# aras-p/UnityGaussianSplatting

Measured on AMD Instinct MI355X. Metric: Msplats/s rendered (sort+view+composite+resolve), bicycle-sized synthetic 6,131,954 splats, 1200x797, Medium; ms/frame in ms_per_step, higher is better.
Workload: dtype f32; 1 GPU; bicycle-sized synthetic 6,131,954 splats, 1200x797, Medium; sort_mode=visible_in_flight, frames_in_flight=2, frames_in_flight_impl=library, splats=6131954, views=1, views_per_rank=1, blend=exact, sort_nth_frame=1, tile_pairs_P=4376060, tile=32x16, visible_splats=1563698, parallelism=single GPU, rccl_ranks=0

## Files before the change

### unitygaussiansplatting_amd/csrc/gs_device_math.h

```cpp
#pragma once
#include <stdint.h>

#if defined(__HIPCC__)
#include <hip/hip_runtime.h>
#include <hip/hip_fp16.h>
#define GS_HD __host__ __device__ __forceinline__
#else
#include <cmath>
#include <cstring>
#define GS_HD inline
#endif

#ifndef GS_CULL_EXTENT
#define GS_CULL_EXTENT 2.8285f
#endif

namespace gsm {

struct AssetView {
    const uint8_t* pos;
    const uint8_t* other;
    const uint8_t* color;
    const uint8_t* sh;
    const uint8_t* chunk;
// ... 505 lines not shown
                    BoxRec& rec, int& x0, int& x1, int& y0, int& y1) {
    const float det = Inverse3(B, rec.inv);
    bool ok = finite32(det) && det != 0.0f;
    for (int k = 0; k < 9; ++k) ok = ok && finite32(rec.inv[k]);
    if (!ok || !(al > 0.0f)) return false;
    const float dx = rc.ox - c[0], dy = rc.oy - c[1], dz = rc.oz - c[2];
    for (int k = 0; k < 3; ++k) rec.lo[k] = fmaf(rec.inv[k * 3 + 2], dz, fmaf(rec.inv[k * 3 + 1], dy, rec.inv[k * 3] * dx));
    rec.r = r; rec.g = g; rec.b = bl; rec.a = det < 0.0f ? -al : al;
    float minx = 3.0e38f, maxx = -3.0e38f, miny = 3.0e38f, maxy = -3.0e38f;
    bool behind = false;
    for (int corner = 0; corner < 8; ++corner) {
        const float lx = (corner & 1) ? 1.0f : -1.0f, ly = (corner & 2) ? 1.0f : -1.0f, lz = (corner & 4) ? 1.0f : -1.0f;
        const float wx = c[0] + fmaf(B[2], lz, fmaf(B[1], ly, B[0] * lx)), wy = c[1] + fmaf(B[5], lz, fmaf(B[4], ly, B[3] * lx)),
                    wz = c[2] + fmaf(B[8], lz, fmaf(B[7], ly, B[6] * lx));
        const float cx = mrow(vp, 0, wx, wy, wz), cy = mrow(vp, 1, wx, wy, wz), cw = mrow(vp, 3, wx, wy, wz);
        if (!(cw > 1.0e-6f)) { behind = true; continue; }
        const float sx = fmaf(0.5f * (cx / cw), rc.W, 0.5f * rc.W), sy = fmaf(-0.5f * (cy / cw), rc.H, 0.5f * rc.H);
        minx = fminf(minx, sx); maxx = fmaxf(maxx, sx); miny = fminf(miny, sy); maxy = fmaxf(maxy, sy);
    }
    if (behind || !(finite32(minx) && finite32(maxx) && finite32(miny) && finite32(maxy))) { x0 = 0; y0 = 0; x1 = (int)rc.W - 1; y1 = (int)rc.H - 1; return true; }
    const float fx0 = fmaxf(floorf(minx) - 1.0f, 0.0f), fx1 = fminf(ceilf(maxx) + 1.0f, rc.W - 1.0f);
    const float fy0 = fmaxf(floorf(miny) - 1.0f, 0.0f), fy1 = fminf(ceilf(maxy) + 1.0f, rc.H - 1.0f);
    if (!(fx0 <= fx1 && fy0 <= fy1)) return false;
    x0 = (int)fx0; x1 = (int)fx1; y0 = (int)fy0; y1 = (int)fy1;
    return true;
}

GS_HD bool IsSplatCut(const EditView& e, float px, float py, float pz) {
    bool finalCut = false;
    for (uint32_t i = 0; i < e.cutoutCount; ++i) {
        const uint32_t* c = e.cutouts + i * 17u;
        const uint32_t tf = c[16];
        const uint32_t type = tf & 0xFFu;
        if (type == 0xFFu) continue;
        const bool invert = (tf & 0xFF00u) != 0;
        float m[12];
#pragma unroll
        for (int k = 0; k < 12; ++k) m[k] = u2f(c[k]);
        const float cx = mrow(m, 0, px, py, pz), cy = mrow(m, 1, px, py, pz), cz = mrow(m, 2, px, py, pz);
        if (type == 0u) { if (dot3f(cx, cy, cz, cx, cy, cz) <= 1.0f) return invert; }
        if (type == 1u) { if (fabsf(cx) <= 1.0f && fabsf(cy) <= 1.0f && fabsf(cz) <= 1.0f) return invert; }
        finalCut = finalCut || !invert;
    }
    return finalCut;
}

struct ViewPartial {
    ViewData view;
    V4 col;
    V3 shMin, shMax;
    float wx, wy, wz;
    uint64_t otherEnd;
    bool shLerp;
    bool front;
    bool culled;
};

GS_HD void CalcViewGeom(const AssetView& a, const FrameConsts& P, const EditView& E, uint32_t idx, ViewPartial& vp, bool allowCull = false,
                        bool outputsOnlyIfDrawn = false) {
    ViewData& view = vp.view;
    if (!outputsOnlyIfDrawn) {
        view.pos[0] = view.pos[1] = view.pos[2] = view.pos[3] = 0.0f;
        view.axis1[0] = view.axis1[1] = view.axis2[0] = view.axis2[1] = 0.0f;
        view.color[0] = view.color[1] = 0u;
        vp.shLerp = false; vp.otherEnd = 0u;
        vp.shMin = { 0, 0, 0 }; vp.shMax = { 0, 0, 0 }; vp.col = { 0, 0, 0, 0 };
    }
    vp.front = false; vp.culled = false;

    V3 pos = LoadVec(a.pos, (uint64_t)idx * vecStride(a.posFmt), a.posFmt);
    const uint32_t ci = idx >> 8;
    const bool chunked = ci < a.chunkCount;
    ChunkRaw ck;
    if (chunked) {
        ck = LoadChunk(a.chunk, ci);
        pos.x = lerpf(u2f(ck.w[4]), u2f(ck.w[5]), pos.x);
        pos.y = lerpf(u2f(ck.w[6]), u2f(ck.w[7]), pos.y);
        pos.z = lerpf(u2f(ck.w[8]), u2f(ck.w[9]), pos.z);
    }
    const float wx = mrow(P.o2w, 0, pos.x, pos.y, pos.z), wy = mrow(P.o2w, 1, pos.x, pos.y, pos.z), wz = mrow(P.o2w, 2, pos.x, pos.y, pos.z);
    vp.wx = wx; vp.wy = wy; vp.wz = wz;
    view.pos[0] = mrow(P.vp, 0, wx, wy, wz);
    view.pos[1] = mrow(P.vp, 1, wx, wy, wz);
    view.pos[2] = mrow(P.vp, 2, wx, wy, wz);
    view.pos[3] = mrow(P.vp, 3, wx, wy, wz);
    if (E.deletedBits && ((E.deletedBits[idx >> 5] >> (idx & 31u)) & 1u)) view.pos[3] = 0.0f;
    if (E.cutoutCount && IsSplatCut(E, pos.x, pos.y, pos.z)) view.pos[3] = 0.0f;
    if (view.pos[3] <= 0.0f) return;
    vp.front = true;

    uint32_t otherStride = 4 + vecStride(a.scaleFmt);
    if (a.shFmt > 3) otherStride += 2;
    const uint64_t otherAddr = (uint64_t)idx * otherStride;
    vp.otherEnd = otherAddr + otherStride;
    V3 scale = LoadVec(a.other, otherAddr + 4, a.scaleFmt);
    if (chunked) {
        scale.x = lerpf(f16tof32(ck.w[10]), f16tof32(ck.w[10] >> 16), scale.x);
        scale.y = lerpf(f16tof32(ck.w[11]), f16tof32(ck.w[11] >> 16), scale.y);
        scale.z = lerpf(f16tof32(ck.w[12]), f16tof32(ck.w[12] >> 16), scale.z);
        scale.x *= scale.x; scale.y *= scale.y; scale.z *= scale.z;
        scale.x *= scale.x; scale.y *= scale.y; scale.z *= scale.z;
        scale.x *= scale.x; scale.y *= scale.y; scale.z *= scale.z;
    }
    const float ss2 = P.splatScale * P.splatScale;

    float vx = mrow(P.mv, 0, pos.x, pos.y, pos.z), vy = mrow(P.mv, 1, pos.x, pos.y, pos.z);
    const float vz = mrow(P.mv, 2, pos.x, pos.y, pos.z);
    const float limX = P.limX, limY = P.limY, focal = P.focal;
    const float rz = 1.0f / vz;
    vx = fminf(fmaxf(vx * rz, -limX), limX) * vz;
    vy = fminf(fmaxf(vy * rz, -limY), limY) * vz;
    const float rzz = rz * rz;
    const float J00 = focal * rz, J02 = -(focal * vx) * rzz;
    const float J11 = J00, J12 = -(focal * vy) * rzz;
    const float T00 = fmaf(J02, P.mv[8], J00 * P.mv[0]), T01 = fmaf(J02, P.mv[9], J00 * P.mv[1]), T02 = fmaf(J02, P.mv[10], J00 * P.mv[2]);
    const float T10 = fmaf(J12, P.mv[8], J11 * P.mv[4]), T11 = fmaf(J12, P.mv[9], J11 * P.mv[5]), T12 = fmaf(J12, P.mv[10], J11 * P.mv[6]);

    if (allowCull) {
        const float w = view.pos[3];
        if (!(w >= P.nearClip && w <= P.farClip)) { vp.culled = true; return; }
        const float smax = fmaxf(fmaxf(fabsf(scale.x), fabsf(scale.y)), fabsf(scale.z));
        const float t2 = dot3f(T00, T01, T02, T00, T01, T02) + dot3f(T10, T11, T12, T10, T11, T12);
        const float lam = fmaf(t2 * (1.1f * ss2), smax * smax, 0.6f);
#if defined(__HIP_DEVICE_COMPILE__)
        const float rad = fmaf(GS_CULL_EXTENT * 1.05f, __builtin_amdgcn_sqrtf(2.0f * lam), 2.0f);
#else
        const float rad = fmaf(GS_CULL_EXTENT * 1.05f, sqrtf(2.0f * lam), 2.0f);
#endif
        const float invw = 1.0f / w;
        const float cx = fmaf(0.5f * (view.pos[0] * invw), P.screenW, 0.5f * P.screenW);
        const float cy = fmaf(-0.5f * (view.pos[1] * invw), P.screenH, 0.5f * P.screenH);
        if (cx - rad > P.screenW || cx + rad < 0.0f || cy - rad > P.screenH || cy + rad < 0.0f) { vp.culled = true; return; }
    }

    const V4 q = DecodeRotation(LoadUInt(a.other, otherAddr));

    V4 col = LoadColorTexel(a, idx);

    if (chunked) {
        col.x = lerpf(f16tof32(ck.w[0]), f16tof32(ck.w[0] >> 16), col.x);
        col.y = lerpf(f16tof32(ck.w[1]), f16tof32(ck.w[1] >> 16), col.y);
        col.z = lerpf(f16tof32(ck.w[2]), f16tof32(ck.w[2] >> 16), col.z);
        col.w = lerpf(f16tof32(ck.w[3]), f16tof32(ck.w[3] >> 16), col.w);
        col.w = InvSquareCentered01(col.w);
        vp.shMin = { f16tof32(ck.w[13]), f16tof32(ck.w[14]), f16tof32(ck.w[15]) };
        vp.shMax = { f16tof32(ck.w[13] >> 16), f16tof32(ck.w[14] >> 16), f16tof32(ck.w[15] >> 16) };
        vp.shLerp = a.shFmt > 0 && a.shFmt <= 3;
    } else {
        vp.shLerp = false; vp.shMin = { 0, 0, 0 }; vp.shMax = { 0, 0, 0 };
    }
    vp.col = col;

    const float x = q.x, y = q.y, z = q.z, w = q.w;
    const float r00 = fmaf(-2.0f, y * y + z * z, 1.0f), r01 = 2.0f * fmaf(x, y, -(w * z)), r02 = 2.0f * fmaf(x, z, w * y);
    const float r10 = 2.0f * fmaf(x, y, w * z), r11 = fmaf(-2.0f, fmaf(x, x, z * z), 1.0f), r12 = 2.0f * fmaf(y, z, -(w * x));
    const float r20 = 2.0f * fmaf(x, z, -(w * y)), r21 = 2.0f * fmaf(y, z, w * x), r22 = fmaf(-2.0f, fmaf(x, x, y * y), 1.0f);
    const float m00 = r00 * scale.x, m01 = r01 * scale.y, m02 = r02 * scale.z;
    const float m10 = r10 * scale.x, m11 = r11 * scale.y, m12 = r12 * scale.z;
    const float m20 = r20 * scale.x, m21 = r21 * scale.y, m22 = r22 * scale.z;
    const float c00 = dot3f(m00, m01, m02, m00, m01, m02) * ss2, c01 = dot3f(m00, m01, m02, m10, m11, m12) * ss2, c02 = dot3f(m00, m01, m02, m20, m21, m22) * ss2;
    const float c11 = dot3f(m10, m11, m12, m10, m11, m12) * ss2, c12 = dot3f(m10, m11, m12, m20, m21, m22) * ss2, c22 = dot3f(m20, m21, m22, m20, m21, m22) * ss2;

    const float VT00 = dot3f(c00, c01, c02, T00, T01, T02), VT01 = dot3f(c00, c01, c02, T10, T11, T12);
    const float VT10 = dot3f(c01, c11, c12, T00, T01, T02), VT11 = dot3f(c01, c11, c12, T10, T11, T12);
    const float VT20 = dot3f(c02, c12, c22, T00, T01, T02), VT21 = dot3f(c02, c12, c22, T10, T11, T12);
    const float cov00 = dot3f(T00, T01, T02, VT00, VT10, VT20) + 0.3f;
    const float cov01 = dot3f(T00, T01, T02, VT01, VT11, VT21);
    const float cov11 = dot3f(T10, T11, T12, VT01, VT11, VT21) + 0.3f;

    const float mid = 0.5f * (cov00 + cov11);
    const float hx = (cov00 - cov11) / 2.0f;
    const float radius = sqrtf(dot2f(hx, cov01, hx, cov01));
    const float lambda1 = mid + radius;
    const float lambda2 = fmaxf(mid - radius, 0.1f);
    float dvx = cov01, dvy = lambda1 - cov00;
    const float invLen = 1.0f / sqrtf(dot2f(dvx, dvy, dvx, dvy));
    dvx *= invLen; dvy *= invLen;
    dvy = -dvy;
    const float s1 = fminf(sqrtf(2.0f * lambda1), 4096.0f), s2 = fminf(sqrtf(2.0f * lambda2), 4096.0f);
    view.axis1[0] = s1 * dvx; view.axis1[1] = s1 * dvy;
    view.axis2[0] = s2 * dvy; view.axis2[1] = s2 * (-dvx);

    const float al = fminf(col.w * P.opacityScale, 65000.0f);
    view.color[1] = f32tof16(al);
}

template <class SHSource>
GS_HD void CalcViewColor(const AssetView& a, const FrameConsts& P, uint32_t idx, ViewPartial& vp, SHSource& shsrc) {
    ViewData& view = vp.view;
    const V4 col = vp.col;
    const V3 shMin = vp.shMin, shMax = vp.shMax;
    const bool shLerp = vp.shLerp;
    const float wx = vp.wx, wy = vp.wy, wz = vp.wz;
    const float dwx = P.camx - wx, dwy = P.camy - wy, dwz = P.camz - wz;
    float ox = mrow3(P.w2o, 0, dwx, dwy, dwz), oy = mrow3(P.w2o, 1, dwx, dwy, dwz), oz = mrow3(P.w2o, 2, dwx, dwy, dwz);
    const float invN = 1.0f / sqrtf(dot3f(ox, oy, oz, ox, oy, oz));
    ox *= invN; oy *= invN; oz *= invN;
    const float dx = -ox, dy = -oy, dz = -oz;

    const bool onlySH = P.shOnly != 0;
    F2 rg = onlySH ? F2{ 0.5f, 0.5f } : F2{ col.x, col.y };
    float b = onlySH ? 0.5f : col.z;
    if (P.shOrder >= 1) {
        uint32_t shIndex = idx;
        if (a.shFmt > 3) shIndex = LoadUShort(a.other, vp.otherEnd - 2);
        shsrc.begin(a.sh + (uint64_t)shIndex * shStrideOf(a.shFmt), a.shFmt);
        const F2 minRG = { shMin.x, shMin.y }, dRG = F2{ shMax.x, shMax.y } - minRG;
        const float minB = shMin.z, dB = shMax.z - shMin.z;
        auto SHK = [&](int k) -> RGB {
            RGB s = shsrc.load_rgb(k);
            if (shLerp) { s.rg = fma2(s.rg, dRG, minRG); s.b = fmaf(s.b, dB, minB); }
            return s;
        };
        auto MUL = [](float w, const RGB& s) -> RGB { return { F2{ w, w } * s.rg, w * s.b }; };
        auto FMA = [](float w, const RGB& s, const RGB& acc) -> RGB { return { fma2(F2{ w, w }, s.rg, acc.rg), fmaf(w, s.b, acc.b) }; };
        {
            const RGB s1v = SHK(1), s2v = SHK(2), s3v = SHK(3);
            RGB t = MUL(dy, RGB{ -s1v.rg, -s1v.b });
            t = FMA(dz, s2v, t);
            t = FMA(dx, RGB{ -s3v.rg, -s3v.b }, t);
            rg = fma2(F2{ GS_SH_C1, GS_SH_C1 }, t.rg, rg); b = fmaf(GS_SH_C1, t.b, b);
        }
        if (P.shOrder >= 2) {
            const float xx = dx * dx, yy = dy * dy, zz = dz * dz;
            const float xy = dx * dy, yz = dy * dz, xz = dx * dz;
            {
                const float b4 = 1.0925484f * xy, b5 = -1.0925484f * yz, b6 = 0.3153916f * (fmaf(2.0f, zz, -xx) - yy),
                            b7 = -1.0925484f * xz, b8 = 0.5462742f * (xx - yy);
                RGB acc = MUL(b4, SHK(4));
                acc = FMA(b5, SHK(5), acc);
                acc = FMA(b6, SHK(6), acc);
                acc = FMA(b7, SHK(7), acc);
                acc = FMA(b8, SHK(8), acc);
                rg += acc.rg; b += acc.b;
            }
            if (P.shOrder >= 3) {
                const float b9 = (-0.5900436f * dy) * fmaf(3.0f, xx, -yy);
                const float b10 = (2.8906114f * xy) * dz;
                const float b11 = (-0.4570458f * dy) * (fmaf(4.0f, zz, -xx) - yy);
                const float b12 = (0.3731763f * dz) * (fmaf(2.0f, zz, -3.0f * xx) - 3.0f * yy);
                const float b13 = (-0.4570458f * dx) * (fmaf(4.0f, zz, -xx) - yy);
                const float b14 = (1.4453057f * dz) * (xx - yy);
                const float b15 = (-0.5900436f * dx) * fmaf(-3.0f, yy, xx);
                RGB acc = MUL(b9, SHK(9));
                acc = FMA(b10, SHK(10), acc);
// ... 37 lines not shown
constexpr uint32_t kAlphaWindowLo = kAlphaThresholdBits - kAlphaWindow / 2u;
GS_HD float Exp2Det(float y) {
    const float n = rintf(y);
    const float f = y - n;
    float p = 1.525273380405984e-05f;
    p = fmaf(p, f, 1.5403530393381608e-04f);
    p = fmaf(p, f, 1.3333558146428443e-03f);
    p = fmaf(p, f, 9.618129107628477e-03f);
    p = fmaf(p, f, 5.550410866482158e-02f);
    p = fmaf(p, f, 2.402265069591007e-01f);
    p = fmaf(p, f, 6.931471805599453e-01f);
    p = fmaf(p, f, 1.0f);
    return ldexpf(p, (int)n);
}
GS_HD float DecideAlpha(float alphaNative, float y, float a, bool& live) {
    const uint32_t u = f2u(alphaNative) - kAlphaWindowLo;
    if (u < kAlphaWindow) {
        const float ad = fminf(fmaxf(Exp2Det(y) * a, 0.0f), 1.0f);
        live = ad >= u2f(kAlphaThresholdBits);
        return ad;
    }
    live = (int32_t)u >= (int32_t)kAlphaWindow;
    return alphaNative;
}

GS_HD float LogDet(float x) {
    const uint32_t u = f2u(x);
    float e = (float)((int)(u >> 23) - 127);
    float m = u2f((u & 0x7fffffu) | 0x3f800000u);
    if (m > 1.41421356f) { m *= 0.5f; e += 1.0f; }
    const float t = (m - 1.0f) / (m + 1.0f);
    const float t2 = t * t;
    const float p = fmaf(t2, fmaf(t2, fmaf(t2, 1.0f / 7.0f, 0.2f), 1.0f / 3.0f), 1.0f);
    return fmaf(e, 0.69314718f, (2.0f * t) * p);
}

GS_HD bool BlockMayTouch(float bcx, float bcy, float half, float cx, float cy, float u1x, float u1y, float u2x, float u2y, float r2) {
    const float dx = bcx - cx, dy = bcy - cy;
    const float d1 = fabsf(fmaf(dy, u1y, dx * u1x)) - half * (fabsf(u1x) + fabsf(u1y));
    const float d2 = fabsf(fmaf(dy, u2y, dx * u2x)) - half * (fabsf(u2x) + fabsf(u2y));
    const float m1 = fmaxf(d1, 0.0f), m2 = fmaxf(d2, 0.0f);
    return (m1 <= 2.001f) && (m2 <= 2.001f) && (fmaf(m2, m2, m1 * m1) <= r2);
}

struct SplatFootprint {
    float cx, cy;
    int x0, x1, y0, y1;
};
GS_HD void PackPixelRect(const SplatFootprint& fp, uint32_t& rx, uint32_t& ry) {
    rx = (uint32_t)fp.x0 | ((uint32_t)fp.y0 << 16);
    ry = (uint32_t)(fp.x1 + 1) | ((uint32_t)(fp.y1 + 1) << 16);
}

GS_HD bool PrepareSplat(const ViewData& v, float W, float H, float nearClip, float farClip, SplatFootprint& fp) {
    fp.x0 = 1; fp.x1 = 0; fp.y0 = 1; fp.y1 = 0; fp.cx = 0.0f; fp.cy = 0.0f;
    const float w = v.pos[3];
    const float a = f16tof32(v.color[1]);
    const int drawable = (int)(w > 0.0f) & (int)(w >= nearClip) & (int)(w <= farClip) & (int)finite32(v.axis1[0]) & (int)finite32(v.axis1[1]) &
                         (int)finite32(v.axis2[0]) & (int)finite32(v.axis2[1]) & (int)(a >= 1.0f / 255.0f);
    if (!drawable) return false;
    const float invw = 1.0f / w;
    const float cx = fmaf(0.5f * (v.pos[0] * invw), W, 0.5f * W);
    const float cy = fmaf(-0.5f * (v.pos[1] * invw), H, 0.5f * H);
    const float a1x = v.axis1[0], a1y = v.axis1[1], a2x = v.axis2[0], a2y = v.axis2[1];
    const float d1 = dot2f(a1x, a1y, a1x, a1y), d2 = dot2f(a2x, a2y, a2x, a2y);
    const int inv1ok = (int)((f2u(d1) - 0x00200001u) <= (0x7f800000u - 0x00200001u)), inv2ok = (int)((f2u(d2) - 0x00200001u) <= (0x7f800000u - 0x00200001u));
    fp.cx = cx; fp.cy = cy;
    if (!((int)finite32(cx) & (int)finite32(cy) & inv1ok & inv2ok)) return false;
    const float exr = 2.0f * (fabsf(a1x) + fabsf(a2x)), eyr = 2.0f * (fabsf(a1y) + fabsf(a2y));
    const float slack = 0.01f;
    int x0, x1, y0, y1;
    PixRange(fp.cx, exr + slack, W, x0, x1);
    PixRange(fp.cy, eyr + slack, H, y0, y1);
    if (x0 > x1 || y0 > y1) return false;
    const float r2 = fmaf(LogDet(255.0f * a), 1.0001f, 1.0e-3f);
    const float rr = sqrtf(fmaxf(r2, 0.0f));
    const float exe = rr * sqrtf(dot2f(a1x, a2x, a1x, a2x)), eye = rr * sqrtf(dot2f(a1y, a2y, a1y, a2y));
    PixRange(fp.cx, fminf(exr, exe) + slack, W, x0, x1);
    PixRange(fp.cy, fminf(eyr, eye) + slack, H, y0, y1);
    if (x0 > x1 || y0 > y1) return true;
    fp.x0 = x0; fp.x1 = x1; fp.y0 = y0; fp.y1 = y1;
    return true;
}

}
```

### unitygaussiansplatting_amd/csrc/gs_raster.hip

```cpp
#include "gs_common.h"
#include <cstdlib>

namespace gs {

namespace {

struct RasterConsts {
    float W, H, nearClip, farClip;
    uint32_t tilesX, tilesY, width, height;
};

constexpr unsigned long long BFLAG_AGG = 1ull << 62, BFLAG_INCL = 2ull << 62, BVAL_MASK = (1ull << 62) - 1ull;
constexpr uint32_t BIN_SPIN_LIMIT = 1u << 24;

__device__ __forceinline__ float rl(float x, int b) { return __int_as_float(__builtin_amdgcn_readlane(__float_as_int(x), b)); }

__device__ __forceinline__ uint32_t wave_incl_scan_u32(uint32_t v) {
#define GS_DPP(x, ctrl, rowmask) (uint32_t)__builtin_amdgcn_update_dpp(0, (int)(x), ctrl, rowmask, 0xf, false)
    v += GS_DPP(v, 0x111, 0xf);
    v += GS_DPP(v, 0x112, 0xf);
    v += GS_DPP(v, 0x114, 0xf);
    v += GS_DPP(v, 0x118, 0xf);
    v += GS_DPP(v, 0x142, 0xa);
    v += GS_DPP(v, 0x143, 0xc);
// ... 599 lines not shown
        for (uint32_t t = tid; t < kBinTileCounters; t += kEmitThreads) {
            const uint32_t c = s_tile[t];
            if (c) {
                atomicAdd(&s_hist[t & digitMask], c);
                if (PASSES >= 2) atomicAdd(&s_hist[256 + ((t >> digitBits) & digitMask)], c);
            }
        }
        __syncthreads();
    }
    uint32_t* myHist = pairHist + (bid % histCopies) * (uint32_t)kHistStride;
    for (int j = tid; j < PASSES * 256; j += kEmitThreads) {
        const uint32_t c = s_hist[j];
        if (c) atomicAdd(&myHist[j], c);
    }
}

__global__ __launch_bounds__(256) void tile_ranges_kernel(const uint32_t* __restrict__ pairKeys, const uint32_t* nPtr,
                                                          uint32_t* __restrict__ tileStart, uint32_t* __restrict__ tileEnd, uint32_t numTiles) {
    GS_CHAIN_PRIORITY();
    const uint32_t n = *nPtr;
    const uint32_t octs = (n + 7u) >> 3;
    for (uint32_t q = blockIdx.x * 256u + threadIdx.x; q < octs; q += gridDim.x * 256u) {
        const uint32_t j0 = q << 3;
        const uint4 ka = ((const uint4*)pairKeys)[2u * q], kb = ((const uint4*)pairKeys)[2u * q + 1u];
        const uint32_t k[10] = { j0 ? pairKeys[j0 - 1u] : 0xffffffffu, ka.x, ka.y, ka.z, ka.w, kb.x, kb.y, kb.z, kb.w,
                                 (j0 + 8u < n) ? pairKeys[j0 + 8u] : 0xffffffffu };
#pragma unroll
        for (int c = 0; c < 8; ++c) {
            const uint32_t j = j0 + (uint32_t)c;
            if (j >= n) break;
            const uint32_t t = k[c + 1];
            if (t >= numTiles) continue;
            if (j == 0 || k[c] != t) tileStart[t] = j;
            if (j == n - 1 || k[c + 2] != t) tileEnd[t] = j + 1;
        }
    }
}

__device__ __forceinline__ float mix_mul_lo(uint32_t h, float x) {
    float d;
    asm("v_fma_mix_f32 %0, %1, %2, 0 op_sel_hi:[1,0,0]" : "=v"(d) : "v"(h), "v"(x));
    return d;
}
__device__ __forceinline__ float mix_mul_hi(uint32_t h, float x) {
    float d;
    asm("v_fma_mix_f32 %0, %1, %2, 0 op_sel:[1,0,0] op_sel_hi:[1,0,0]" : "=v"(d) : "v"(h), "v"(x));
    return d;
}
__device__ __forceinline__ float mix_mul_lo_sat_after_trans(uint32_t h, float x) {
    float d;
    asm("s_nop 0\n\tv_fma_mix_f32 %0, %1, %2, 0 op_sel_hi:[1,0,0] clamp" : "=v"(d) : "v"(h), "v"(x));
    return d;
}
__device__ __forceinline__ float mix_one_minus_hi(uint32_t h) {
    float d;
    asm("v_fma_mix_f32 %0, %1, -1.0, 1.0 op_sel:[1,0,0] op_sel_hi:[1,0,0]" : "=v"(d) : "v"(h));
    return d;
}
__device__ __forceinline__ void mix_blend4(uint32_t& rg, uint32_t& ba, float pr, float pg, float pb, float pa, float t) {
    asm("v_fma_mixlo_f16 %0, %2, %6, %0 op_sel_hi:[0,0,1]\n\t"
        "v_fma_mixlo_f16 %1, %4, %6, %1 op_sel_hi:[0,0,1]\n\t"
        "v_fma_mixhi_f16 %0, %3, %6, %0 op_sel:[0,0,1] op_sel_hi:[0,0,1]\n\t"
        "v_fma_mixhi_f16 %1, %5, %6, %1 op_sel:[0,0,1] op_sel_hi:[0,0,1]"
        : "+v"(rg), "+v"(ba) : "v"(pr), "v"(pg), "v"(pb), "v"(pa), "v"(t));
}

__device__ __forceinline__ float half_lo(uint32_t u) { return (float)__builtin_bit_cast(_Float16, (unsigned short)(u & 0xffffu)); }
__device__ __forceinline__ float half_hi(uint32_t u) { return (float)__builtin_bit_cast(_Float16, (unsigned short)(u >> 16)); }
template <int MODE> struct PixelAcc;
template <> struct PixelAcc<0> {
    uint32_t rg, ba;
    __device__ __forceinline__ void load(uint2 d) { rg = d.x; ba = d.y; }
    __device__ __forceinline__ void blend(uint32_t c0, uint32_t c1, float alpha) {
        const float t = mix_one_minus_hi(ba);
        mix_blend4(rg, ba, mix_mul_hi(c0, alpha), mix_mul_lo(c0, alpha), mix_mul_hi(c1, alpha), alpha, t);
    }
    __device__ __forceinline__ void blend_src(float pr, float pg, float pb, float pa) { const float t = mix_one_minus_hi(ba); mix_blend4(rg, ba, pr, pg, pb, pa, t); }
    __device__ __forceinline__ bool finished() const { return (ba >> 16) == 0x3c00u; }
    __device__ __forceinline__ bool saturated() const { return false; }
    __device__ __forceinline__ uint2 pack() const { return make_uint2(rg, ba); }
};
template <> struct PixelAcc<1> {
    float r, g, b, a;
    __device__ __forceinline__ void load(uint2 d) {
        r = gsm::f16tof32(d.x); g = gsm::f16tof32(d.x >> 16); b = gsm::f16tof32(d.y); a = gsm::f16tof32(d.y >> 16);
    }
    __device__ __forceinline__ void blend(uint32_t c0, uint32_t c1, float alpha) {
        const float t = 1.0f - a;
        r = fmaf(mix_mul_hi(c0, alpha), t, r); g = fmaf(mix_mul_lo(c0, alpha), t, g); b = fmaf(mix_mul_hi(c1, alpha), t, b);
        a = fmaf(alpha, t, a);
    }
    __device__ __forceinline__ void blend_src(float pr, float pg, float pb, float pa) { const float t = 1.0f - a; r = fmaf(pr, t, r); g = fmaf(pg, t, g); b = fmaf(pb, t, b); a = fmaf(pa, t, a); }
    __device__ __forceinline__ bool finished() const { return (1.0f - a) < (1.0f / 4096.0f); }
    __device__ __forceinline__ bool saturated() const { return (1.0f - a) < (1.0f / 4096.0f); }
    __device__ __forceinline__ uint2 pack() const {
        uint2 o;
        o.x = gsm::f32tof16(r) | (gsm::f32tof16(g) << 16);
        o.y = gsm::f32tof16(b) | (gsm::f32tof16(a) << 16);
        return o;
    }
};

typedef uint32_t u4v __attribute__((ext_vector_type(4)));

#ifdef GS_BLEND_STATS
__device__ unsigned long long g_blendStats[8];
#define GS_STAT(i, v) do { if (lane == 0) atomicAdd(&g_blendStats[i], (unsigned long long)(v)); } while (0)
#else
#define GS_STAT(i, v) do { } while (0)
#endif
#ifdef GS_BLEND_TL
__device__ unsigned long long g_blendTl[8192 * 8];
#endif
template <int MODE, bool DEPTH, int TWL, int THL>
__global__ __launch_bounds__(64 << (TWL + THL - 6)) void blend_kernel(const uint32_t* __restrict__ pairVals, const uint32_t* __restrict__ tileStart,
                                                    const uint32_t* __restrict__ tileEnd, const uint32_t* __restrict__ tileOrder,
                                                    uint32_t* __restrict__ tileCost, const SplatRec* __restrict__ recs,
                                                    uint16_t* __restrict__ rt, RasterConsts rc, int dstIsZero,
                                                    const float* __restrict__ recW, const float* __restrict__ sceneDepth,
                                                    const BinControl* __restrict__ binCtl, const uint32_t* __restrict__ pairSortError,
                                                    FrameReport* __restrict__ report) {
    constexpr int TW = 1 << TWL, TH = 1 << THL;
    constexpr int NWX = TW / 8, NW = NWX * (TH / 8);
    constexpr int NT = 64 * NW;
    constexpr uint32_t SLOTS = 2048u * 256u / (uint32_t)NT;
    __shared__ float4 s_a[NT];
    __shared__ uint4 s_b[NT];
    __shared__ float4 s_e[NT];
    __shared__ int s_done;
    __shared__ uint32_t s_cost;
    uint32_t survWalked = 0;

    const int tid = threadIdx.x, lane = tid & 63, w = tid >> 6;
#ifdef GS_BLEND_TL
    const unsigned long long tl0 = wall_clock64();
#endif
    if (blockIdx.x == 0 && tid == 0) write_report(binCtl, pairSortError, report, (uint32_t)TWL | ((uint32_t)THL << 8));
    const uint32_t tile = tileOrder[blockIdx.x];
#ifndef GS_BLEND_NOPRIO
    if (blockIdx.x < SLOTS / 8u) __builtin_amdgcn_s_setprio(3);
    else if (blockIdx.x < 3u * SLOTS / 8u) __builtin_amdgcn_s_setprio(2);
    else if (blockIdx.x < 6u * SLOTS / 8u) __builtin_amdgcn_s_setprio(1);
#endif
    const uint32_t tx = tile % rc.tilesX, ty = tile / rc.tilesX;
    const uint32_t start = tileStart[tile], end = tileEnd[tile];
    const int qx0 = (int)tx * TW + (w % NWX) * 8, qy0 = (int)ty * TH + (w / NWX) * 8;
    const int px = qx0 + (lane & 7), py = qy0 + (lane >> 3);
    const bool inside = px < (int)rc.width && py < (int)rc.height;
    uint2* dst = (uint2*)(rt + ((size_t)py * rc.width + (size_t)px) * 4);
    if (start >= end) {
        if (threadIdx.x == 0) tileCost[tile] = 0;
#ifdef GS_BLEND_TL
        if (threadIdx.x == 0 && blockIdx.x < 8192u) { unsigned long long* q = g_blendTl + blockIdx.x * 8u; q[0] = tl0; q[1] = wall_clock64(); q[2] = 0; q[3] = 0; q[4] = 0; q[5] = tile; q[6] = 0; }
#endif
        if (dstIsZero && inside) *dst = make_uint2(0u, 0u);
        return;
    }
    uint32_t batchesWalked = 0;

    const float fx = (float)px + 0.5f, fy = (float)py + 0.5f;
    const gsm::F2 fxy = { fx, fy };
    const float qminx = (float)qx0 + 0.5f, qmaxx = (float)qx0 + 7.5f, qminy = (float)qy0 + 0.5f, qmaxy = (float)qy0 + 7.5f;

    PixelAcc<MODE> acc;
    float sceneZ = 0.0f;
    if (DEPTH) sceneZ = inside ? sceneDepth[(size_t)py * rc.width + (size_t)px] : 0.0f;
    acc.load((inside && !dstIsZero) ? *dst : make_uint2(0u, 0u));
    if (tid == 0) s_done = 0;
    if (tid == 0) s_cost = 0u;
    bool waveDone = false;

    const uint32_t lastPair = end - 1u;
    float4 r0, r1;
    float rw = 0.0f;
    {
        const uint32_t s0 = pairVals[min(start + (uint32_t)tid, lastPair)];
        const float4* rp = (const float4*)(recs + s0);
        r0 = rp[0]; r1 = rp[1];
        if (DEPTH) rw = recW[s0];
    }
    uint32_t sidxNext = pairVals[min(start + (uint32_t)NT + (uint32_t)tid, lastPair)];
    for (uint32_t bs = start; bs < end; bs += (uint32_t)NT) {
        __syncthreads();
        if (s_done == NW) break;
        ++batchesWalked;
        GS_STAT(0, 1);
        const uint32_t cnt = min((uint32_t)NT, end - bs);
        if ((uint32_t)tid < cnt) {
            const float inv1 = 1.0f / gsm::dot2f(r0.z, r0.w, r0.z, r0.w);
            const float inv2 = 1.0f / gsm::dot2f(r1.x, r1.y, r1.x, r1.y);
            const float ca = gsm::f16tof32(gsm::f2u(r1.w));
            const float exr = 2.0f * (fabsf(r0.z) + fabsf(r1.x)), eyr = 2.0f * (fabsf(r0.w) + fabsf(r1.y));
            const float r2 = fmaf(gsm::LogDet(255.0f * ca), 1.0001f, 1.0e-3f);
            const float rr = sqrtf(fmaxf(r2, 0.0f));
            const float exe = rr * sqrtf(gsm::dot2f(r0.z, r1.x, r0.z, r1.x)), eye = rr * sqrtf(gsm::dot2f(r0.w, r1.y, r0.w, r1.y));
            s_a[tid] = make_float4(r0.x, r0.y, r0.z * inv1, r1.x * inv2);
            s_b[tid] = make_uint4(gsm::f2u(r0.w * inv1), gsm::f2u(r1.y * inv2), gsm::f2u(r1.z), gsm::f2u(r1.w));
            s_e[tid] = make_float4(fminf(exr, exe) + 0.02f, fminf(eyr, eye) + 0.02f, r2, rw);
        }
        {
            const float4* rp = (const float4*)(recs + sidxNext);
            r0 = rp[0]; r1 = rp[1];
            if (DEPTH) rw = recW[sidxNext];
            sidxNext = pairVals[min(bs + 2u * (uint32_t)NT + (uint32_t)tid, lastPair)];
        }
        __syncthreads();
        if (!waveDone) {
            for (uint32_t c = 0; c < cnt; c += 64u) {
                const uint32_t j = c + lane;
                bool hit = false;
                GS_STAT(1, 1);
                if (j < cnt) {
                    const float4 ra = s_a[j];
                    const float4 re = s_e[j];
                    hit = (ra.x + re.x >= qminx) && (ra.x - re.x <= qmaxx) && (ra.y + re.y >= qminy) && (ra.y - re.y <= qmaxy);
#ifdef GS_BLEND_STATS
                    { const unsigned long long bb = __ballot(hit); if (__ffsll((long long)__ballot(true)) - 1 == lane) atomicAdd(&g_blendStats[2], (unsigned long long)__popcll(bb)); }
#endif
                    const uint4 rb = s_b[j];
                    hit = hit && gsm::BlockMayTouch((float)qx0 + 4.0f, (float)qy0 + 4.0f, 3.5f, ra.x, ra.y, ra.z, gsm::u2f(rb.x), ra.w, gsm::u2f(rb.y), re.z);
                }
                unsigned long long mask = __ballot(hit);
                survWalked += (uint32_t)__popcll(mask);
                auto fragment = [&](const float4 A4, const u4v B4, const uint32_t rec) {
                    const gsm::F2 d = fxy - gsm::F2{ A4.x, A4.y };
                    const gsm::F2 q = gsm::fma2(gsm::F2{ d.y, d.y }, gsm::F2{ gsm::u2f(B4.x), gsm::u2f(B4.y) }, gsm::F2{ d.x, d.x } * gsm::F2{ A4.z, A4.w });
                    const float q1 = q.x, q2 = q.y;
                    const float power = -fmaf(q2, q2, q1 * q1);
                    const float y2 = power * 1.44269504088896340736f;
                    float alpha = mix_mul_lo_sat_after_trans(B4.w, __builtin_amdgcn_exp2f(y2));
                    const int inQuad = (int)(fmaxf(fabsf(q1), fabsf(q2)) <= 2.0f);
                    bool live;
                    if (MODE == 0) {
                        const bool geHi = alpha >= gsm::u2f(gsm::kAlphaWindowLo + gsm::kAlphaWindow);
                        const bool geLo = alpha >= gsm::u2f(gsm::kAlphaWindowLo);
                        live = (inQuad & (int)geHi) != 0;
                        const bool nearT = (inQuad & (int)geLo & (int)!geHi) != 0;
                        if (__builtin_expect(__any(nearT), 0)) {
                            if (nearT) alpha = gsm::DecideAlpha(alpha, y2, half_lo(B4.w), live);
                        }
                    } else {
                        live = (inQuad & (int)(alpha >= 1.0f / 255.0f)) != 0;
                    }
                    if (DEPTH) live = live && (s_e[rec].w <= sceneZ);
                    if (MODE == 1) live = live && !acc.saturated();
#ifdef GS_BLEND_STATS
                    { const unsigned long long lv = __ballot(live); GS_STAT(4, __popcll(lv)); }
#endif
                    if (live) acc.blend(B4.z, B4.w, alpha);
                };
#ifdef GS_BLEND_PREFETCH
                if (mask) {
                    int b0 = __ffsll((long long)mask) - 1;
                    mask &= ~(1ull << b0);
                    float4 A0 = s_a[c + b0];
                    u4v B0 = *(const u4v*)&s_b[c + b0];
                    for (;;) {
                        const bool more1 = mask != 0;
                        const int b1 = more1 ? __ffsll((long long)mask) - 1 : b0;
                        mask &= ~(1ull << b1);
                        const float4 A1 = s_a[c + b1];
                        u4v B1 = *(const u4v*)&s_b[c + b1];
                        asm volatile("" : "+v"(B0));
                        fragment(A0, B0, c + (uint32_t)b0);
                        if (!more1) break;
                        const bool more0 = mask != 0;
                        b0 = more0 ? __ffsll((long long)mask) - 1 : b1;
                        mask &= ~(1ull << b0);
                        A0 = s_a[c + b0];
                        B0 = *(const u4v*)&s_b[c + b0];
                        asm volatile("" : "+v"(B1));
                        fragment(A1, B1, c + (uint32_t)b1);
                        if (!more0) break;
                    }
                }
#else
                while (mask) {
                    const int b = __ffsll((long long)mask) - 1;
                    mask &= ~(1ull << b);
                    const float4 A4 = s_a[c + b];
                    u4v B4 = *(const u4v*)&s_b[c + b];
                    asm volatile("" : "+v"(B4));
                    fragment(A4, B4, c + (uint32_t)b);
                }
#endif
                if (__all(!inside || acc.finished())) {
                    waveDone = true;
                    if (lane == 0) atomicAdd(&s_done, 1);
                    break;
                }
            }
        }
    }
    if (inside) *dst = acc.pack();
    if (lane == 0) atomicMax(&s_cost, survWalked);
    GS_STAT(3, survWalked);
    if (w == 0) GS_STAT(5, 1);
    __syncthreads();
    if (threadIdx.x == 0) tileCost[tile] = min(254u, (s_cost + batchesWalked * (uint32_t)(NT / 8)) / 4u);
#ifdef GS_BLEND_TL
    if (threadIdx.x == 0 && blockIdx.x < 8192u) {
        unsigned long long* q = g_blendTl + blockIdx.x * 8u;
        uint32_t hwid; asm volatile("s_getreg_b32 %0, hwreg(HW_REG_HW_ID)" : "=s"(hwid));
        uint32_t xcc; asm volatile("s_getreg_b32 %0, hwreg(HW_REG_XCC_ID)" : "=s"(xcc));
        q[0] = tl0; q[1] = wall_clock64(); q[2] = batchesWalked; q[3] = s_cost; q[4] = end - start; q[5] = tile; q[6] = hwid | ((unsigned long long)xcc << 32);
    }
#endif
}

__global__ __launch_bounds__(256) void splat_depth_kernel(gsm::AssetView a, gsm::FrameConsts P, const uint32_t* __restrict__ visMask32, float* __restrict__ recW) {
    const uint32_t idx = blockIdx.x * 256u + threadIdx.x;
    if (idx >= a.n || !((visMask32[idx >> 5] >> (idx & 31u)) & 1u)) return;
    const gsm::V3 pos = gsm::LoadSplatPosChunk(a, idx, blockIdx.x);
    const float wx = gsm::mrow(P.o2w, 0, pos.x, pos.y, pos.z), wy = gsm::mrow(P.o2w, 1, pos.x, pos.y, pos.z), wz = gsm::mrow(P.o2w, 2, pos.x, pos.y, pos.z);
    recW[idx] = gsm::mrow(P.vp, 3, wx, wy, wz);
}

template <bool CHUNKS>
__global__ __launch_bounds__(256) void box_setup_kernel(gsm::AssetView a, gsm::FrameConsts P, gsm::RayConsts ray, uint32_t count, gsm::BoxRec* __restrict__ recs,
                                                        uint2* __restrict__ rects, unsigned long long* __restrict__ visMask, uint8_t* __restrict__ waveFlags) {
    const uint32_t idx = blockIdx.x * 256u + threadIdx.x;
    bool visible = false;
    uint2 rect = make_uint2(0u, 0u);
    if (idx < count) {
        float c[3], B[9], r, g, b, al;
        if (!CHUNKS) {
            const gsm::V3 pos = gsm::LoadSplatPos(a, idx);
            gsm::V4 q; gsm::V3 sc; float opacity;
            gsm::LoadSplatRotScaleOpacity(a, idx, q, sc, opacity);
            const float sx = sc.x * P.splatScale, sy = sc.y * P.splatScale, sz = sc.z * P.splatScale;
            for (int k = 0; k < 3; ++k) c[k] = gsm::mrow(P.o2w, k, pos.x, pos.y, pos.z);
            const float x = q.x, y = q.y, z = q.z, w = q.w;
            const float m1[9] = { fmaf(-2.0f, fmaf(z, z, y * y), 1.0f) * sx, (2.0f * fmaf(-w, z, x * y)) * sy, (2.0f * fmaf(w, y, x * z)) * sz,
                                  (2.0f * fmaf(w, z, x * y)) * sx, fmaf(-2.0f, fmaf(z, z, x * x), 1.0f) * sy, (2.0f * fmaf(-w, x, y * z)) * sz,
                                  (2.0f * fmaf(-w, y, x * z)) * sx, (2.0f * fmaf(w, x, y * z)) * sy, fmaf(-2.0f, fmaf(y, y, x * x), 1.0f) * sz };
            for (int i = 0; i < 3; ++i)
// ... 548 lines not shown
```

### unitygaussiansplatting_amd/csrc/gs_view.hip

```cpp
#include "gs_common.h"

namespace gs {

namespace {

template <int FMT> struct SHFromLds {
    const uint32_t* rec;
    __device__ __forceinline__ void begin(const uint8_t*, uint32_t) {}
    __device__ __forceinline__ uint32_t half_at(int h) const { return (rec[h >> 1] >> ((h & 1) * 16)) & 0xffffu; }
    __device__ __forceinline__ gsm::V3 load(int k) const {
        if (FMT == 0) return { gsm::u2f(rec[(k - 1) * 3]), gsm::u2f(rec[(k - 1) * 3 + 1]), gsm::u2f(rec[(k - 1) * 3 + 2]) };
        if (FMT == 2) return gsm::Dec_11_10_11(rec[k - 1]);
        if (FMT == 3) return gsm::Dec_5_6_5(half_at(k - 1));
        return { gsm::f16tof32(half_at((k - 1) * 3)), gsm::f16tof32(half_at((k - 1) * 3 + 1)), gsm::f16tof32(half_at((k - 1) * 3 + 2)) };
    }
    __device__ __forceinline__ gsm::RGB load_rgb(int k) const {
        if (FMT == 3) {
            const uint32_t e = half_at(k - 1);
            return { gsm::F2{ (float)(e & 31), (float)((e >> 5) & 63) } * gsm::F2{ GS_R31, GS_R63 }, (float)((e >> 11) & 31) * GS_R31 };
        }
        const gsm::V3 v = load(k);
        return { gsm::F2{ v.x, v.y }, v.z };
    }
};
// ... 11 lines not shown
    constexpr int REC = sh_rec_dwords(SHMODE < 4 ? SHMODE : 3);
    constexpr int STRIDE = REC | 1;
    constexpr int SH_DW = SHMODE < 4 ? 256 * STRIDE : 0;
    constexpr int NVEC = (REC * 256 / 4 + 255) / 256;
    __shared__ uint4 s_stage[cmax(SH_DW, FULL ? 256 * 10 : 4) / 4 + 1];
    __shared__ int s_any;
    uint32_t* s_dw = (uint32_t*)s_stage;
    const uint32_t base = blockIdx.x * 256u;
    const uint32_t idx = base + threadIdx.x;
    const uint32_t cnt = min(256u, a.n - base);
    const uint32_t totalDw = cnt * (uint32_t)REC, totalVec = totalDw >> 2;
    const uint32_t* shSrc = (const uint32_t*)(a.sh + (size_t)base * (REC * 4));

    uint4 shv[SHMODE < 4 ? NVEC : 1];
    uint32_t shTail = 0;
    auto sh_issue = [&]() {
#pragma unroll
        for (int it = 0; it < NVEC; ++it) {
            const uint32_t j = (uint32_t)it * 256u + threadIdx.x;
            shv[it] = make_uint4(0u, 0u, 0u, 0u);
            if (j < totalVec) shv[it] = ((const uint4*)shSrc)[j];
        }
        if ((totalDw & 3u) && threadIdx.x < (totalDw & 3u)) shTail = shSrc[(totalVec << 2) + threadIdx.x];
    };
    auto sh_park = [&]() {
#pragma unroll
        for (int it = 0; it < NVEC; ++it) {
            const uint32_t j = (uint32_t)it * 256u + threadIdx.x;
            if (j < totalVec) {
                const uint32_t d = j << 2;
                const uint32_t v[4] = { shv[it].x, shv[it].y, shv[it].z, shv[it].w };
                if (REC % 4 == 0) {
                    const uint32_t r = d / (uint32_t)REC, o = d - r * (uint32_t)REC;
#pragma unroll
                    for (int c = 0; c < 4; ++c) s_dw[r * STRIDE + o + c] = v[c];
                } else {
#pragma unroll
                    for (int c = 0; c < 4; ++c) { const uint32_t dd = d + c, r = dd / (uint32_t)REC; s_dw[r * STRIDE + (dd - r * (uint32_t)REC)] = v[c]; }
                }
            }
        }
        if ((totalDw & 3u) && threadIdx.x < (totalDw & 3u)) { const uint32_t dd = (totalVec << 2) + threadIdx.x, r = dd / (uint32_t)REC; s_dw[r * STRIDE + (dd - r * (uint32_t)REC)] = shTail; }
    };
    auto shade = [&](gsm::ViewPartial& vp) {
        if (SHMODE < 4) {
            SHFromLds<SHMODE < 4 ? SHMODE : 3> src;
            src.rec = s_dw + threadIdx.x * STRIDE;
            gsm::CalcViewColor(a, P, idx, vp, src);
        } else {
            gsm::SHFromBlob src;
            gsm::CalcViewColor(a, P, idx, vp, src);
        }
    };

    gsm::ViewPartial vp;
    gsm::SplatFootprint fp;
    uint2 rect = make_uint2(0u, 0u);
    bool visible = false;
    const bool shStaged = SHMODE < 4;

    if (FULL) {
        if (shStaged) { sh_issue(); sh_park(); __syncthreads(); }
        if (idx < a.n) {
            gsm::CalcViewGeom(a, P, E, idx, vp);
            if (vp.front) shade(vp);
            const bool ok = gsm::PrepareSplat(vp.view, P.screenW, P.screenH, P.nearClip, P.farClip, fp);
            visible = ok && fp.x0 <= fp.x1;
        }
    } else {
        if (P.cullOn && blockIdx.x < a.chunkCount) {
            const uint32_t m = gsm::ChunkCornerOutside(a, P, blockIdx.x, threadIdx.x & 7u);
            bool outside = false;
#pragma unroll
            for (int pl = 0; pl < 6; ++pl) outside = outside || __all((m >> pl) & 1u);
            if (outside) {
                if (idx < a.n) rects[idx] = make_uint2(0u, 0u);
                if ((threadIdx.x & 63u) == 0u && idx < a.n) visMask[idx >> 6] = 0ull;
                if ((threadIdx.x & 63u) == 0u && idx < a.n) wave_flags_of(visMask, a.n)[idx >> 6] = 0u;
                return;
            }
        }
        if (threadIdx.x == 0) s_any = 0;
        if (idx < a.n) {
            gsm::CalcViewGeom(a, P, E, idx, vp, true, true);
            const bool ok = vp.front && !vp.culled && gsm::PrepareSplat(vp.view, P.screenW, P.screenH, P.nearClip, P.farClip, fp);
            visible = ok && fp.x0 <= fp.x1;
        }
        __syncthreads();
        if (__any(visible) && (threadIdx.x & 63u) == 0u) s_any = 1;
        __syncthreads();
        if (s_any) {
            if (shStaged) { sh_issue(); sh_park(); __syncthreads(); }
            if (visible) shade(vp);
        }
    }

    if (idx < a.n) {
        if (visible) {
            gsm::PackPixelRect(fp, rect.x, rect.y);
            uint4* rp = (uint4*)(recs + idx);
            rp[0] = make_uint4(gsm::f2u(fp.cx), gsm::f2u(fp.cy), gsm::f2u(vp.view.axis1[0]), gsm::f2u(vp.view.axis1[1]));
            rp[1] = make_uint4(gsm::f2u(vp.view.axis2[0]), gsm::f2u(vp.view.axis2[1]), vp.view.color[0], vp.view.color[1]);
        }
        rects[idx] = rect;
    }
    const unsigned long long vb = __ballot(visible);
    if ((threadIdx.x & 63u) == 0u && (idx < a.n)) visMask[idx >> 6] = vb;
    if ((threadIdx.x & 63u) == 0u && (idx < a.n)) wave_flags_of(visMask, a.n)[idx >> 6] = vb != 0ull ? 1u : 0u;
    if (!FULL) return;

    if (shStaged) __syncthreads();
    if (idx < a.n) {
        const gsm::ViewData& v = vp.view;
        uint32_t* o = s_dw + threadIdx.x * 10;
        o[0] = gsm::f2u(v.pos[0]); o[1] = gsm::f2u(v.pos[1]); o[2] = gsm::f2u(v.pos[2]); o[3] = gsm::f2u(v.pos[3]);
        o[4] = gsm::f2u(v.axis1[0]); o[5] = gsm::f2u(v.axis1[1]); o[6] = gsm::f2u(v.axis2[0]); o[7] = gsm::f2u(v.axis2[1]);
        o[8] = v.color[0]; o[9] = v.color[1];
    }
    __syncthreads();
    {
        const uint32_t dwords = cnt * 10u;
        uint32_t* g = (uint32_t*)(out + base);
        const uint32_t vec = dwords / 4u;
        for (uint32_t j = threadIdx.x; j < vec; j += 256u) ((uint4*)g)[j] = s_stage[j];
        for (uint32_t j = vec * 4u + threadIdx.x; j < dwords; j += 256u) g[j] = s_dw[j];
    }
}

}

void flatten_params(const gs_frame_params* p, gsm::FrameConsts& c) {
    memcpy(c.mv, p->matrix_mv, 12 * sizeof(float));
    memcpy(c.o2w, p->matrix_object_to_world, 12 * sizeof(float));
    memcpy(c.w2o, p->matrix_world_to_object, 12 * sizeof(float));
    memcpy(c.vp, p->matrix_vp, 16 * sizeof(float));
    gsm::FrameConstsFromProjection(c, p->proj_m00, p->proj_m11, p->screen_w); c.screenW = p->screen_w; c.screenH = p->screen_h;
    c.camx = p->cam_pos_world[0]; c.camy = p->cam_pos_world[1]; c.camz = p->cam_pos_world[2];
    c.splatScale = p->splat_scale; c.opacityScale = p->opacity_scale;
    c.shOrder = p->sh_order; c.shOnly = p->sh_only;
    c.nearClip = p->near_clip; c.farClip = p->far_clip;
    gsm::FrameConstsChunkCull(c);
}

template <bool FULL>
static void launch_calc_view(int mode, uint32_t grid, hipStream_t st, const gsm::AssetView& a, const gsm::FrameConsts& c, const gsm::EditView& e,
                             const ViewOutputs& o) {
// ... 22 lines not shown
```

Baseline: 15730 Msplats/s.

## Stage blend records as pre-split f32 and specialize view shading per chunk

```diff
diff --git a/unitygaussiansplatting_amd/csrc/gs_device_math.h b/unitygaussiansplatting_amd/csrc/gs_device_math.h
--- a/unitygaussiansplatting_amd/csrc/gs_device_math.h
+++ b/unitygaussiansplatting_amd/csrc/gs_device_math.h
@@ -581,12 +581,13 @@
     float wx, wy, wz;
     uint64_t otherEnd;
     bool shLerp;
+    float invw;
     bool front;
     bool culled;
 };
 
-GS_HD void CalcViewGeom(const AssetView& a, const FrameConsts& P, const EditView& E, uint32_t idx, ViewPartial& vp, bool allowCull = false,
-                        bool outputsOnlyIfDrawn = false) {
+GS_HD void CalcViewGeomChunk(const AssetView& a, const FrameConsts& P, const EditView& E, uint32_t idx, uint32_t ci, ViewPartial& vp, bool allowCull,
+                             bool outputsOnlyIfDrawn) {
     ViewData& view = vp.view;
     if (!outputsOnlyIfDrawn) {
         view.pos[0] = view.pos[1] = view.pos[2] = view.pos[3] = 0.0f;
@@ -598,7 +599,6 @@
     vp.front = false; vp.culled = false;
 
     V3 pos = LoadVec(a.pos, (uint64_t)idx * vecStride(a.posFmt), a.posFmt);
-    const uint32_t ci = idx >> 8;
     const bool chunked = ci < a.chunkCount;
     ChunkRaw ck;
     if (chunked) {
@@ -657,6 +657,7 @@
         const float rad = fmaf(GS_CULL_EXTENT * 1.05f, sqrtf(2.0f * lam), 2.0f);
 #endif
         const float invw = 1.0f / w;
+        vp.invw = invw;
         const float cx = fmaf(0.5f * (view.pos[0] * invw), P.screenW, 0.5f * P.screenW);
         const float cy = fmaf(-0.5f * (view.pos[1] * invw), P.screenH, 0.5f * P.screenH);
         if (cx - rad > P.screenW || cx + rad < 0.0f || cy - rad > P.screenH || cy + rad < 0.0f) { vp.culled = true; return; }
@@ -714,12 +715,19 @@
     view.color[1] = f32tof16(al);
 }
 
-template <class SHSource>
+GS_HD void CalcViewGeom(const AssetView& a, const FrameConsts& P, const EditView& E, uint32_t idx, ViewPartial& vp, bool allowCull = false,
+                        bool outputsOnlyIfDrawn = false) {
+    CalcViewGeomChunk(a, P, E, idx, idx >> 8, vp, allowCull, outputsOnlyIfDrawn);
+}
+
+GS_HD bool ChunkLerpsSH(const AssetView& a, uint32_t ci) { return ci < a.chunkCount && a.shFmt > 0 && a.shFmt <= 3; }
+
+template <int LERP = -1, class SHSource>
 GS_HD void CalcViewColor(const AssetView& a, const FrameConsts& P, uint32_t idx, ViewPartial& vp, SHSource& shsrc) {
     ViewData& view = vp.view;
     const V4 col = vp.col;
     const V3 shMin = vp.shMin, shMax = vp.shMax;
-    const bool shLerp = vp.shLerp;
+    const bool shLerp = LERP < 0 ? vp.shLerp : (LERP != 0);
     const float wx = vp.wx, wy = vp.wy, wz = vp.wz;
     const float dwx = P.camx - wx, dwy = P.camy - wy, dwz = P.camz - wz;
     float ox = mrow3(P.w2o, 0, dwx, dwy, dwz), oy = mrow3(P.w2o, 1, dwx, dwy, dwz), oz = mrow3(P.w2o, 2, dwx, dwy, dwz);
@@ -863,14 +871,14 @@
     ry = (uint32_t)(fp.x1 + 1) | ((uint32_t)(fp.y1 + 1) << 16);
 }
 
-GS_HD bool PrepareSplat(const ViewData& v, float W, float H, float nearClip, float farClip, SplatFootprint& fp) {
+GS_HD bool PrepareSplat(const ViewData& v, float W, float H, float nearClip, float farClip, SplatFootprint& fp, const float* invwKnown = nullptr) {
     fp.x0 = 1; fp.x1 = 0; fp.y0 = 1; fp.y1 = 0; fp.cx = 0.0f; fp.cy = 0.0f;
     const float w = v.pos[3];
     const float a = f16tof32(v.color[1]);
     const int drawable = (int)(w > 0.0f) & (int)(w >= nearClip) & (int)(w <= farClip) & (int)finite32(v.axis1[0]) & (int)finite32(v.axis1[1]) &
                          (int)finite32(v.axis2[0]) & (int)finite32(v.axis2[1]) & (int)(a >= 1.0f / 255.0f);
     if (!drawable) return false;
-    const float invw = 1.0f / w;
+    const float invw = invwKnown ? *invwKnown : 1.0f / w;
     const float cx = fmaf(0.5f * (v.pos[0] * invw), W, 0.5f * W);
     const float cy = fmaf(-0.5f * (v.pos[1] * invw), H, 0.5f * H);
     const float a1x = v.axis1[0], a1y = v.axis1[1], a2x = v.axis2[0], a2y = v.axis2[1];
diff --git a/unitygaussiansplatting_amd/csrc/gs_raster.hip b/unitygaussiansplatting_amd/csrc/gs_raster.hip
--- a/unitygaussiansplatting_amd/csrc/gs_raster.hip
+++ b/unitygaussiansplatting_amd/csrc/gs_raster.hip
@@ -675,6 +675,16 @@
     asm("s_nop 0\n\tv_fma_mix_f32 %0, %1, %2, 0 op_sel_hi:[1,0,0] clamp" : "=v"(d) : "v"(h), "v"(x));
     return d;
 }
+__device__ __forceinline__ float fma_zero(float a, float x) {
+    float d;
+    asm("v_fma_f32 %0, %1, %2, 0" : "=v"(d) : "v"(a), "v"(x));
+    return d;
+}
+__device__ __forceinline__ float fma_zero_sat_after_trans(float a, float x) {
+    float d;
+    asm("s_nop 0\n\tv_fma_f32 %0, %1, %2, 0 clamp" : "=v"(d) : "v"(a), "v"(x));
+    return d;
+}
 __device__ __forceinline__ float mix_one_minus_hi(uint32_t h) {
     float d;
     asm("v_fma_mix_f32 %0, %1, -1.0, 1.0 op_sel:[1,0,0] op_sel_hi:[1,0,0]" : "=v"(d) : "v"(h));
@@ -725,6 +735,8 @@
 };
 
 typedef uint32_t u4v __attribute__((ext_vector_type(4)));
+typedef float f2v __attribute__((ext_vector_type(2)));
+typedef float f4v __attribute__((ext_vector_type(4)));
 
 #ifdef GS_BLEND_STATS
 __device__ unsigned long long g_blendStats[8];
@@ -748,7 +760,12 @@
     constexpr int NT = 64 * NW;
     constexpr uint32_t SLOTS = 2048u * 256u / (uint32_t)NT;
     __shared__ float4 s_a[NT];
+#ifdef GS_BLEND_STAGE_F16
     __shared__ uint4 s_b[NT];
+#else
+    __shared__ float4 s_b[NT];
+    __shared__ float4 s_c[NT];
+#endif
     __shared__ float4 s_e[NT];
     __shared__ int s_done;
     __shared__ uint32_t s_cost;
@@ -818,7 +835,12 @@
             const float rr = sqrtf(fmaxf(r2, 0.0f));
             const float exe = rr * sqrtf(gsm::dot2f(r0.z, r1.x, r0.z, r1.x)), eye = rr * sqrtf(gsm::dot2f(r0.w, r1.y, r0.w, r1.y));
             s_a[tid] = make_float4(r0.x, r0.y, r0.z * inv1, r1.x * inv2);
+#ifdef GS_BLEND_STAGE_F16
             s_b[tid] = make_uint4(gsm::f2u(r0.w * inv1), gsm::f2u(r1.y * inv2), gsm::f2u(r1.z), gsm::f2u(r1.w));
+#else
+            *(float2*)&s_b[tid] = make_float2(r0.w * inv1, r1.y * inv2);
+            s_c[tid] = make_float4(half_hi(gsm::f2u(r1.z)), half_lo(gsm::f2u(r1.z)), half_hi(gsm::f2u(r1.w)), half_lo(gsm::f2u(r1.w)));
+#endif
             s_e[tid] = make_float4(fminf(exr, exe) + 0.02f, fminf(eyr, eye) + 0.02f, r2, rw);
         }
         {
@@ -840,18 +862,42 @@
 #ifdef GS_BLEND_STATS
                     { const unsigned long long bb = __ballot(hit); if (__ffsll((long long)__ballot(true)) - 1 == lane) atomicAdd(&g_blendStats[2], (unsigned long long)__popcll(bb)); }
 #endif
-                    const uint4 rb = s_b[j];
-                    hit = hit && gsm::BlockMayTouch((float)qx0 + 4.0f, (float)qy0 + 4.0f, 3.5f, ra.x, ra.y, ra.z, gsm::u2f(rb.x), ra.w, gsm::u2f(rb.y), re.z);
+#ifdef GS_BLEND_STAGE_F16
+                    const uint4 rbu = s_b[j];
+                    const float2 rb = make_float2(gsm::u2f(rbu.x), gsm::u2f(rbu.y));
+#else
+                    const float2 rb = *(const float2*)&s_b[j];
+#endif
+                    hit = hit && gsm::BlockMayTouch((float)qx0 + 4.0f, (float)qy0 + 4.0f, 3.5f, ra.x, ra.y, ra.z, rb.x, ra.w, rb.y, re.z);
                 }
                 unsigned long long mask = __ballot(hit);
                 survWalked += (uint32_t)__popcll(mask);
-                auto fragment = [&](const float4 A4, const u4v B4, const uint32_t rec) {
+#ifdef GS_BLEND_STAGE_F16
+                struct Staged { float4 A; u4v B; };
+                auto staged = [&](const uint32_t rec) -> Staged { return { s_a[rec], *(const u4v*)&s_b[rec] }; };
+                auto pin = [](Staged& S) { asm volatile("" : "+v"(S.B)); };
+#else
+                struct Staged { float4 A; f2v B; f4v C; };
+                auto staged = [&](const uint32_t rec) -> Staged { return { s_a[rec], *(const f2v*)&s_b[rec], *(const f4v*)&s_c[rec] }; };
+                auto pin = [](Staged& S) { asm volatile("" : "+v"(S.B), "+v"(S.C)); };
+#endif
+                auto fragment = [&](const Staged& S, const uint32_t rec) {
+                    const float4 A4 = S.A;
+#ifdef GS_BLEND_STAGE_F16
+                    const float u1y = gsm::u2f(S.B.x), u2y = gsm::u2f(S.B.y);
+#else
+                    const float u1y = S.B.x, u2y = S.B.y;
+#endif
                     const gsm::F2 d = fxy - gsm::F2{ A4.x, A4.y };
-                    const gsm::F2 q = gsm::fma2(gsm::F2{ d.y, d.y }, gsm::F2{ gsm::u2f(B4.x), gsm::u2f(B4.y) }, gsm::F2{ d.x, d.x } * gsm::F2{ A4.z, A4.w });
+                    const gsm::F2 q = gsm::fma2(gsm::F2{ d.y, d.y }, gsm::F2{ u1y, u2y }, gsm::F2{ d.x, d.x } * gsm::F2{ A4.z, A4.w });
                     const float q1 = q.x, q2 = q.y;
                     const float power = -fmaf(q2, q2, q1 * q1);
                     const float y2 = power * 1.44269504088896340736f;
-                    float alpha = mix_mul_lo_sat_after_trans(B4.w, __builtin_amdgcn_exp2f(y2));
+#ifdef GS_BLEND_STAGE_F16
+                    float alpha = mix_mul_lo_sat_after_trans(S.B.w, __builtin_amdgcn_exp2f(y2));
+#else
+                    float alpha = fma_zero_sat_after_trans(S.C.w, __builtin_amdgcn_exp2f(y2));
+#endif
                     const int inQuad = (int)(fmaxf(fabsf(q1), fabsf(q2)) <= 2.0f);
                     bool live;
                     if (MODE == 0) {
@@ -860,7 +906,11 @@
                         live = (inQuad & (int)geHi) != 0;
                         const bool nearT = (inQuad & (int)geLo & (int)!geHi) != 0;
                         if (__builtin_expect(__any(nearT), 0)) {
-                            if (nearT) alpha = gsm::DecideAlpha(alpha, y2, half_lo(B4.w), live);
+#ifdef GS_BLEND_STAGE_F16
+                            if (nearT) alpha = gsm::DecideAlpha(alpha, y2, half_lo(S.B.w), live);
+#else
+                            if (nearT) alpha = gsm::DecideAlpha(alpha, y2, S.C.w, live);
+#endif
                         }
                     } else {
                         live = (inQuad & (int)(alpha >= 1.0f / 255.0f)) != 0;
@@ -870,30 +920,31 @@
 #ifdef GS_BLEND_STATS
                     { const unsigned long long lv = __ballot(live); GS_STAT(4, __popcll(lv)); }
 #endif
-                    if (live) acc.blend(B4.z, B4.w, alpha);
+#ifdef GS_BLEND_STAGE_F16
+                    if (live) acc.blend(S.B.z, S.B.w, alpha);
+#else
+                    if (live) acc.blend_src(fma_zero(S.C.x, alpha), fma_zero(S.C.y, alpha), fma_zero(S.C.z, alpha), alpha);
+#endif
                 };
 #ifdef GS_BLEND_PREFETCH
                 if (mask) {
                     int b0 = __ffsll((long long)mask) - 1;
                     mask &= ~(1ull << b0);
-                    float4 A0 = s_a[c + b0];
-                    u4v B0 = *(const u4v*)&s_b[c + b0];
+                    Staged S0 = staged(c + (uint32_t)b0);
                     for (;;) {
                         const bool more1 = mask != 0;
                         const int b1 = more1 ? __ffsll((long long)mask) - 1 : b0;
                         mask &= ~(1ull << b1);
-                        const float4 A1 = s_a[c + b1];
-                        u4v B1 = *(const u4v*)&s_b[c + b1];
-                        asm volatile("" : "+v"(B0));
-                        fragment(A0, B0, c + (uint32_t)b0);
+                        Staged S1 = staged(c + (uint32_t)b1);
+                        pin(S0);
+                        fragment(S0, c + (uint32_t)b0);
                         if (!more1) break;
                         const bool more0 = mask != 0;
                         b0 = more0 ? __ffsll((long long)mask) - 1 : b1;
                         mask &= ~(1ull << b0);
-                        A0 = s_a[c + b0];
-                        B0 = *(const u4v*)&s_b[c + b0];
-                        asm volatile("" : "+v"(B1));
-                        fragment(A1, B1, c + (uint32_t)b1);
+                        S0 = staged(c + (uint32_t)b0);
+                        pin(S1);
+                        fragment(S1, c + (uint32_t)b1);
                         if (!more0) break;
                     }
                 }
@@ -901,10 +952,9 @@
                 while (mask) {
                     const int b = __ffsll((long long)mask) - 1;
                     mask &= ~(1ull << b);
-                    const float4 A4 = s_a[c + b];
-                    u4v B4 = *(const u4v*)&s_b[c + b];
-                    asm volatile("" : "+v"(B4));
-                    fragment(A4, B4, c + (uint32_t)b);
+                    Staged S = staged(c + (uint32_t)b);
+                    pin(S);
+                    fragment(S, c + (uint32_t)b);
                 }
 #endif
                 if (__all(!inside || acc.finished())) {
diff --git a/unitygaussiansplatting_amd/csrc/gs_view.hip b/unitygaussiansplatting_amd/csrc/gs_view.hip
--- a/unitygaussiansplatting_amd/csrc/gs_view.hip
+++ b/unitygaussiansplatting_amd/csrc/gs_view.hip
@@ -87,6 +87,16 @@
             gsm::CalcViewColor(a, P, idx, vp, src);
         }
     };
+    auto shade_uniform = [&](gsm::ViewPartial& vp, const bool lerp) {
+        if (SHMODE < 4) {
+            SHFromLds<SHMODE < 4 ? SHMODE : 3> src;
+            src.rec = s_dw + threadIdx.x * STRIDE;
+            if (lerp) gsm::CalcViewColor<1>(a, P, idx, vp, src); else gsm::CalcViewColor<0>(a, P, idx, vp, src);
+        } else {
+            gsm::SHFromBlob src;
+            if (lerp) gsm::CalcViewColor<1>(a, P, idx, vp, src); else gsm::CalcViewColor<0>(a, P, idx, vp, src);
+        }
+    };
 
     gsm::ViewPartial vp;
     gsm::SplatFootprint fp;
@@ -117,8 +127,13 @@
         }
         if (threadIdx.x == 0) s_any = 0;
         if (idx < a.n) {
+#ifdef GS_VIEW_PER_SPLAT_FLAGS
             gsm::CalcViewGeom(a, P, E, idx, vp, true, true);
             const bool ok = vp.front && !vp.culled && gsm::PrepareSplat(vp.view, P.screenW, P.screenH, P.nearClip, P.farClip, fp);
+#else
+            gsm::CalcViewGeomChunk(a, P, E, idx, blockIdx.x, vp, true, true);
+            const bool ok = vp.front && !vp.culled && gsm::PrepareSplat(vp.view, P.screenW, P.screenH, P.nearClip, P.farClip, fp, &vp.invw);
+#endif
             visible = ok && fp.x0 <= fp.x1;
         }
         __syncthreads();
@@ -126,7 +141,11 @@
         __syncthreads();
         if (s_any) {
             if (shStaged) { sh_issue(); sh_park(); __syncthreads(); }
+#ifdef GS_VIEW_PER_SPLAT_FLAGS
             if (visible) shade(vp);
+#else
+            if (visible) shade_uniform(vp, gsm::ChunkLerpsSH(a, blockIdx.x));
+#endif
         }
     }
 
```

After: 15310 Msplats/s. 0.973x the previous value.
